# lh3/minimap2

Hardware: NVIDIA H100
Metric: aligned bases/sec (map-ont, 10 kb reads) (higher is better)
Workload: dtype int8 DP cells (int32 scores), u64 hashes, f32 chain penalties

## Files before the change

### include/mm_b200.h

```cpp
#ifndef MM_B200_H
#define MM_B200_H

#include <stdint.h>
#include <stddef.h>
#include "minimap.h"

#ifdef __cplusplus
extern "C" {
#endif

typedef struct mmb_ctx_s mmb_ctx_t;

int  mmb_device_count(void);
mmb_ctx_t *mmb_ctx_create(int device);
void mmb_ctx_destroy(mmb_ctx_t *ctx);
void *mmb_ctx_stream(mmb_ctx_t *ctx);
uint64_t mmb_launch_count(mmb_ctx_t *ctx, int reset);
void  mmb_profile_enable(mmb_ctx_t *ctx, int on);
double mmb_profile_ms(mmb_ctx_t *ctx, int which, int reset);
uint64_t mmb_profile_units(mmb_ctx_t *ctx, int which, int reset);

#define MMB_KSW_SCORE_ONLY   0x01
#define MMB_KSW_RIGHT        0x02
#define MMB_KSW_GENERIC_SC   0x04
// ... 23 lines not shown
} mmb_ksw_job_t;

typedef struct {
	int32_t max, zdropped;
	int32_t max_q, max_t;
	int32_t mqe, mqe_t;
	int32_t mte, mte_q;
	int32_t score;
	int32_t n_cigar, reach_end;
	uint32_t cigar_off;
	int32_t zd_max, zd_t0, zd_t1, zd_q0, zd_q1;
} mmb_ksw_res_t;

typedef struct {
	int8_t mat[25];
	int8_t q, e, q2, e2;
	int8_t noncan, junc_bonus, junc_pen;
	int16_t zd_skip;
} mmb_ksw_score_t;

int64_t mmb_ksw_batch_host(mmb_ctx_t *ctx, const mmb_ksw_score_t *sc, int n_jobs, const mmb_ksw_job_t *jobs,
						   const uint8_t *query, int64_t query_len, const uint8_t *target, int64_t target_len,
						   mmb_ksw_res_t *res, uint32_t *cigar_buf, int64_t cigar_cap);

int64_t mmb_sketch_batch_host(mmb_ctx_t *ctx, int n_seq, const char *seqs, const int64_t *off, int w, int k, int is_hpc,
							  uint32_t rid0, uint64_t *out_xy , int64_t out_cap, int64_t *n_out);

int mmb_ctx_set_junctions(mmb_ctx_t *ctx, int64_t n, const int64_t *st, const int64_t *en, const int8_t *strand);

int mmb_ctx_set_splice_scores(mmb_ctx_t *ctx, int strand, int64_t n, const int64_t *pos, const uint8_t *val);

typedef struct {
	int32_t max_dist_x, max_dist_y, bw, max_skip, max_iter, min_cnt, min_sc;
	float chn_pen_gap, chn_pen_skip;
	int32_t is_cdna, n_seg;
	int32_t use_rmq, max_dist_inner, rmq_size_cap;
} mmb_chain_par_t;

int mmb_chain_batch_host(mmb_ctx_t *ctx, const mmb_chain_par_t *par, int n_reads, const uint64_t *anchors_xy, const int64_t *a_off,
						 int32_t *n_u, int32_t *n_v, uint64_t *u_out, uint64_t *a_out_xy);
int mmb_chain_rmq_batch_host(mmb_ctx_t *ctx, const mmb_chain_par_t *par, int n_reads, const uint64_t *anchors_xy, const int64_t *a_off,
							 int32_t *n_u, int32_t *n_v, uint64_t *u_out, uint64_t *a_out_xy);

typedef struct {
	int64_t q0;
	int64_t t0;
// ... 57 lines not shown
```

### minimap2_b200/csrc/ksw_extd2.cu

```cuda
#include "mmb_internal.h"
#include "ksw_plan.h"
#include <algorithm>
#include <numeric>
#include <mutex>

#define KSW_NEG_INF (-0x40000000)

namespace {

struct KswArgs {
	const mmb_ksw_job_t *jobs;
	const int *order;
	int n;
	const uint8_t *query;
	const void *target;
	int t_packed;
	mmb_ksw_res_t *res;
	uint32_t *cigar;
	long long cigar_cap;
	unsigned long long *cigar_used;
	uint8_t *pws;
	size_t pws_stride;
	uint32_t *cigws;
	size_t cigws_stride;
// ... 696 lines not shown
		}
		uint64_t c = 0; for (int i : fastj) c += (uint64_t)h_jobs[i].qlen * h_jobs[i].tlen;
		fprintf(stderr, "[ksw] packed path: %zu jobs, cells %.3g; ll %zu\n", fastj.size(), (double)c, llj.size());
	}
	if (!tj[n_tiers].empty() || !tj[2 * n_tiers + 1].empty()) {
		fprintf(stderr, "[ERROR] ksw job longer than %d not supported by this build\n", tiers[n_tiers - 1].maxlen);
		abort();
	}
	if (!llj.empty()) {
		LLArgs L;
		int maxq = 1;
		for (int i : llj) maxq = std::max(maxq, h_jobs[i].qlen);
		L.jobs = d_jobs, L.query = d_query, L.target = d_target, L.t_packed = t_packed, L.res = d_res, L.n = (int)llj.size();
		for (int i = 0; i < 25; ++i) L.mat[i] = sc->mat[i];
		L.slen_max = (maxq + 7) / 8;
		L.ws_stride = ((size_t)L.slen_max * 8 * 2 * 4 + (size_t)L.slen_max * 8 + 255) & ~(size_t)255;
		int groups = std::min((int)llj.size(), ctx->n_sm * 16 * 4);
		int grid = (groups * 8 + 127) / 128;
		groups = grid * 16;
		int *d_order = (int*)ctx->d_g.reserve(((size_t)n_jobs * 3 + 256) * sizeof(int)) + (size_t)n_jobs * 2 + 128;
		L.counter = d_order, L.order = d_order + 1;
		K.ll.pws_bytes = L.ws_stride * (size_t)groups;
		K.ll.order = std::move(llj), K.ll.d_order = d_order;
		K.ll.go = [=](uint8_t *ws, uint32_t *) {
			LLArgs B = L;
			B.ws = (int16_t*)ws;
			ksw_ll_kernel<<<grid, 128, 0, ctx->stream>>>(B);
			MMB_CUDA_CHECK(cudaGetLastError());
			++ctx->n_launch;
		};
	}
	if (ctx->profiling) ctx->prof_bytes[MMB_PROF_KSW] += io_bytes + cells;
	int *d_queues = (int*)ctx->d_g.reserve(((size_t)n_jobs * 3 + 256) * sizeof(int));
	size_t g_off = (size_t)n_jobs + 64;
	std::vector<KswPlan> &plans = K.plans;
	K.cells = cells;
	mmb_ksw_fast_plan(ctx, sc, fastj, h_jobs, d_jobs, d_query, d_target, t_packed, d_res, d_cigar, cigar_cap, d_cigar_used, d_queues, plans);
	for (int pass = 0; pass < 2; ++pass) {
		if (pass == 1) {
			A.q = sc->q, A.e = sc->e, A.q2 = sc->q2, A.e2 = 0;
			A.skip = (-min_sc > 2 * (sc->q + sc->e)) || sc->q2 <= sc->q + sc->e;
			int lt2 = sc->e > 0? (sc->q2 - sc->q) / sc->e - 1 : 0;
			if (sc->q2 > sc->q + sc->e + lt2 * sc->e) ++lt2;
			A.long_thres = lt2, A.long_diff = lt2 * sc->e - (sc->q2 - sc->q);
		}
	for (int k = 0; k < n_tiers; ++k) {
		std::vector<int> &v = tj[pass * (n_tiers + 1) + k];
		if (v.empty()) continue;
		mmb_order_by_cells(v, h_jobs);
		int maxq = 0, maxt = 0; size_t maxp = 0; int maxsum = 0;
// ... 20 lines not shown
				MMB_CUDA_CHECK(cudaFuncSetAttribute(ksw_extd2_kernel<256, true>, cudaFuncAttributeMaxDynamicSharedMemorySize, (int)ctx->smem_optin - 1024));
			});
		}
		void (*kern)(KswArgs) = G == 32? (pass? ksw_extd2_kernel<32, true> : ksw_extd2_kernel<32, false>) : (pass? ksw_extd2_kernel<256, true> : ksw_extd2_kernel<256, false>);
		MMB_CUDA_CHECK(cudaOccupancyMaxActiveBlocksPerMultiprocessor(&cta_per_sm, kern, threads, smem));
		if (smem > ctx->smem_optin - 1024 || cta_per_sm < 1) {
			fprintf(stderr, "[ERROR] ksw tier %d needs %zu B shared memory per CTA\n", k, smem);
			abort();
		}
		int grid = ctx->n_sm * cta_per_sm;
		int need = ((int)v.size() + nw - 1) / nw;
		grid = std::max(1, std::min(grid, need));
		maxp = (maxp + 255) & ~(size_t)255;
		const size_t gws_stride = gstate? (state_bytes + 255) & ~(size_t)255 : 0;
		while ((size_t)grid * nw * (maxp + gws_stride) > ((size_t)2 << 30) && grid > 1) grid = (grid + 1) / 2;
		A.pws_stride = maxp, A.cigws_stride = (size_t)maxsum + 8;
		int *d_order = d_queues + g_off; g_off += v.size() + 1;
		A.counter = d_order, A.order = d_order + 1, A.n = (int)v.size();
		KswPlan pl;
		pl.order = std::move(v), pl.d_order = d_order;
		const size_t pws_area = A.pws_stride * (size_t)grid * nw;
		pl.pws_bytes = pws_area + gws_stride * (size_t)grid * nw, pl.cigws_bytes = A.cigws_stride * 4 * (size_t)grid * nw;
		const KswArgs A0 = A;
		pl.go = [=](uint8_t *pws, uint32_t *cigws) {
			KswArgs B = A0;
			B.pws = pws, B.cigws = cigws;
			B.gws = gstate? pws + pws_area : nullptr, B.gws_stride = gws_stride;
			kern<<<grid, threads, smem, ctx->stream>>>(B);
			MMB_CUDA_CHECK(cudaGetLastError());
			++ctx->n_launch;
		};
		plans.push_back(pl);
	}
	}
}

void mmb_ksw_enqueue(mmb_ctx_t *ctx, const KswLaunch &K)
{
	size_t pws_bytes = K.ll.pws_bytes, cigws_bytes = 0;
	for (const KswPlan &pl : K.plans) pws_bytes = std::max(pws_bytes, pl.pws_bytes), cigws_bytes = std::max(cigws_bytes, pl.cigws_bytes);
	uint8_t *pws = (uint8_t*)ctx->d_e.reserve(pws_bytes);
	uint32_t *cigws = (uint32_t*)ctx->d_f.reserve(cigws_bytes);
	auto upload = [&](const KswPlan &pl) {
		MMB_CUDA_CHECK(cudaMemcpyAsync(pl.d_order + 1, pl.order.data(), pl.order.size() * sizeof(int), cudaMemcpyHostToDevice, ctx->stream));
		MMB_CUDA_CHECK(cudaMemsetAsync(pl.d_order, 0, sizeof(int), ctx->stream));
	};
	if (K.ll.go) {
		upload(K.ll);
		ProfScope prof(ctx, MMB_PROF_OTHER, 0);
		K.ll.go(pws, nullptr);
	}
	for (const KswPlan &pl : K.plans) upload(pl);
	ProfScope prof(ctx, MMB_PROF_KSW, K.cells);
	for (const KswPlan &pl : K.plans) pl.go(pws, cigws);
}

void mmb_ksw_launch(mmb_ctx_t *ctx, const mmb_ksw_score_t *sc, int n_jobs, const mmb_ksw_job_t *h_jobs, const mmb_ksw_job_t *d_jobs,
					const uint8_t *d_query, const void *d_target, int t_packed,
					mmb_ksw_res_t *d_res, uint32_t *d_cigar, int64_t cigar_cap, unsigned long long *d_cigar_used)
{
	if (n_jobs <= 0) return;
	KswLaunch K;
	mmb_ksw_plan(ctx, sc, n_jobs, h_jobs, d_jobs, d_query, d_target, t_packed, d_res, d_cigar, cigar_cap, d_cigar_used, K);
	mmb_ksw_enqueue(ctx, K);
}
```

### minimap2_b200/csrc/ksw_fast.cu

```cuda
#include "mmb_internal.h"
#include "ksw_plan.h"
#include <algorithm>

#define KSW_NEG_INF (-0x40000000)

namespace {

struct FastArgs {
	const mmb_ksw_job_t *jobs;
	const int *order;
	int n;
	const uint8_t *query;
	const void *target;
	int t_packed;
	mmb_ksw_res_t *res;
	uint32_t *cigar;
	long long cigar_cap;
	unsigned long long *cigar_used;
	uint8_t *pws; size_t pws_stride;
	uint32_t *cigws; size_t cigws_stride;
	int *counter;
	int qmax;
	int8_t mch, mis, scn;
	int8_t q, e, q2, e2;
	int qe0;
	int8_t zd_q, zd_e;
	int8_t zd_scn;
	int zd_skip;
	int long_thres, long_diff;
	int8_t mat[25];
	uint32_t one, neg1;
};

__device__ __forceinline__ uint8_t fetch_t(const void *target, int packed, long long idx)
{
	if (packed) {
		const uint32_t *S = (const uint32_t*)target;
		return (uint8_t)(S[idx >> 3] >> ((idx & 7) << 2) & 0xf);
	}
	return ((const uint8_t*)target)[idx];
}

__device__ __forceinline__ void push_cig(uint32_t *cig, int &n, uint32_t op, int len)
{
	if (n == 0 || op != (cig[n - 1] & 0xf)) cig[n++] = (uint32_t)len << 4 | op;
	else cig[n - 1] += (uint32_t)len << 4;
}

template<int C>
__global__ void __launch_bounds__(128) ksw_fast_kernel(FastArgs A)
{
	extern __shared__ __align__(16) uint8_t smem[];
	const int lane = threadIdx.x & 31, wk = threadIdx.x >> 5, nwk = blockDim.x >> 5;
	const int worker = blockIdx.x * nwk + wk;
// ... 157 lines not shown
			if (jj >= 0) push_cig(cig, n, 1, jj + 1);
		}
		n = __shfl_sync(full, n, 0);
		unsigned long long coff = 0;
		if (n > 0) {
			if (lane == 0) coff = atomicAdd(A.cigar_used, (unsigned long long)n);
			coff = __shfl_sync(full, coff, 0);
			const bool rev_cigar = (jb.flag & MMB_KSW_REV_CIGAR) != 0;
			if ((long long)(coff + n) <= A.cigar_cap)
				for (int k = lane; k < n; k += 32) A.cigar[coff + k] = rev_cigar? cig[k] : cig[n - 1 - k];
		}
		if (lane == 0) {
			mmb_ksw_res_t o;
			o.zd_max = -1, o.zd_t0 = o.zd_t1 = o.zd_q0 = o.zd_q1 = -1;
			o.max = 0, o.zdropped = 0, o.max_q = o.max_t = o.mqe_t = o.mte_q = -1, o.mqe = o.mte = KSW_NEG_INF;
			o.score = score, o.n_cigar = n, o.reach_end = 0, o.cigar_off = (uint32_t)coff;
			A.res[jid] = o;
		}
		__syncwarp();
	}
}


#if defined(MMB_EMU) || defined(MMB_PK_NO_FMA)
#define PK_FADD(x, y) ((x) + (y))
#define PK_FSUB(x, y) ((x) - (y))
#else
#define PK_FADD(x, y) pk_mad((x), ONE, (y))
#define PK_FSUB(x, y) pk_mad((y), NEG1, (x))
__device__ __forceinline__ uint32_t pk_mad(uint32_t a, uint32_t b, uint32_t c)
{
	uint32_t d;
	asm("mad.lo.u32 %0, %1, %2, %3;" : "=r"(d) : "r"(a), "r"(b), "r"(c));
	return d;
}
#endif

template<int H, int LN>
#ifndef PK_MINB
#define PK_MINB (H <= 8? 4 : 3)
#endif
__global__ void __launch_bounds__(128, PK_MINB) ksw_pk_kernel(FastArgs A)
{
	extern __shared__ __align__(16) uint8_t smem[];
	constexpr int C = 2 * H;
	constexpr int CPH = H <= 1? 1 : H <= 2? 2 : H <= 4? 4 : H <= 8? 8 : 16;
// ... 6 lines not shown
	const int worker0 = (blockIdx.x * nwk + wk) * NJ;
	uint8_t *qs = smem + (size_t)(wk * NJ + grp) * A.qmax;
	constexpr int TSM = LN * C;
	constexpr int TW = 80, TILE = 32 * TW;
	uint8_t *ts = smem + (size_t)nwk * NJ * A.qmax + (size_t)(wk * NJ + grp) * TSM;
	uint8_t *tile = smem + (size_t)nwk * NJ * (A.qmax + TSM) + (size_t)wk * TILE;
	uint8_t *p = A.pws + A.pws_stride * (size_t)(worker0 + grp);
	const int q = A.q, e = A.e, q2 = A.q2, e2 = A.e2, qe = q + e, qe2 = q2 + e2;
	const unsigned full = 0xffffffffu;
	#define PK_ENC(v) ((uint32_t)((v) + 128) << 8)
	#define PK2(v) (PK_ENC(v) * 0x10001u)
	const uint32_t BB2 = 0x80008000u, CLEAN = 0xff00ff00u;
	const uint32_t TAGS = 0x03040506u, NBB2 = 0u - BB2;
	const uint32_t ONE = A.one, NEG1 = A.neg1;
	(void)ONE; (void)NEG1;
	const uint32_t KX = BB2 - ((uint32_t)e << 8) * 0x10001u - 0x00060006u, KY = BB2 - ((uint32_t)e << 8) * 0x10001u - 0x00050005u;
	const uint32_t KX2 = BB2 - ((uint32_t)e2 << 8) * 0x10001u - 0x00040004u, KY2 = BB2 - ((uint32_t)e2 << 8) * 0x10001u - 0x00030003u;
	const uint32_t NQX = PK2(-qe) | 0x00080008u, NQY = PK2(-qe) | 0x00100010u, NQX2 = PK2(-qe2) | 0x00200020u, NQY2 = PK2(-qe2) | 0x00400040u;
	const uint32_t SCN_T = PK2((int)A.scn) + 0x00070007u;
	const uint32_t KMM = (uint32_t)((int)A.mch - (int)A.mis) << 8;
	const uint32_t E_QE = PK_ENC(-q - e), E_E = PK_ENC(-e), E_E2 = PK_ENC(-e2), E_LD = PK_ENC(A.long_diff), E_QE2 = PK_ENC(-q2 - e2);
	const uint32_t XT0 = E_QE | 6u, YT0 = E_QE | 5u, X2T0 = E_QE2 | 4u, Y2T0 = E_QE2 | 3u;
	const int lt = A.long_thres;

	#pragma unroll 1
	for (;;) {
		int slot = 0;
		if (sub == 0) slot = atomicAdd(A.counter, 1);
		slot = __shfl_sync(full, slot, lead);
		const bool act = slot < A.n;
		if (!__any_sync(full, act)) break;
		int jid = -1, qlen = 0, tlen = 0, jflag = 0;
		mmb_ksw_job_t jb;
		if (act) { jid = A.order[slot]; jb = A.jobs[jid]; qlen = jb.qlen, tlen = jb.tlen, jflag = jb.flag; }
		for (int i = sub; i <= qlen; i += LN) {
			uint8_t c = 4;
			if (i < qlen) {
				c = A.query[jb.q_start + (long long)i * jb.q_step];
				if ((jflag & MMB_JOB_Q_COMP) && c < 4) c = 3 - c;
			}
			qs[i] = c < 4? (uint8_t)(1u << c) : (uint8_t)0x80;
		}
		const int t0 = sub * C;
		uint32_t TBM[H], MSC[H], U[H], Y[H], Y2[H];
		#pragma unroll
		for (int c = 0; c < H; ++c) {
			uint32_t tbm = 0, msc = 0, u = 0;
			#pragma unroll
			for (int h = 0; h < 2; ++h) {
// ... 92 lines not shown
						if constexpr (CPH == 1) *pa = (uint8_t)lo[0];
						else if constexpr (CPH == 2) *(uint16_t*)pa = (uint16_t)lo[0];
						else if constexpr (CPH == 4) *(uint32_t*)pa = lo[0];
						else if constexpr (CPH == 8) *(uint2*)pa = make_uint2(lo[0], lo[NW - 1]);
						else *(uint4*)pa = make_uint4(lo[0], lo[1], lo[2], lo[NW - 1]);
					}
					if (jA >= 1) {
						uint8_t *pb = pa + CPH;
						if constexpr (CPH == 1) *pb = (uint8_t)hi[0];
						else if constexpr (CPH == 2) *(uint16_t*)pb = (uint16_t)hi[0];
						else if constexpr (CPH == 4) *(uint32_t*)pb = hi[0];
						else if constexpr (CPH == 8) *(uint2*)pb = make_uint2(hi[0], hi[NW - 1]);
						else *(uint4*)pb = make_uint4(hi[0], hi[1], hi[2], hi[NW - 1]);
					}
				}
			}
		}
		int score = hrow;
		#pragma unroll
		for (int o = LN / 2; o > 0; o >>= 1) score += __shfl_xor_sync(full, score, o);
		score += (int)(hcol_acc >> 8) - 128 * qlen - A.qe0;
		score = __shfl_sync(full, score, lead);
		__syncwarp();
		#pragma unroll 1
		for (int g = 0; g < NJ; ++g) {
			const int src = g * LN;
			if (!__shfl_sync(full, (int)act, src)) continue;
			const int g_tlen = __shfl_sync(full, tlen, src), g_qlen = __shfl_sync(full, qlen, src), g_jid = __shfl_sync(full, jid, src);
			const int g_flag = __shfl_sync(full, jflag, src), g_score = __shfl_sync(full, score, src);
			const uint8_t *gp = A.pws + A.pws_stride * (size_t)(worker0 + g);
			uint32_t *cig = A.cigws + A.cigws_stride * (size_t)(worker0 + g);
			int n = 0, i = g_tlen - 1, jj = g_qlen - 1, state = 0;
			uint32_t run_op = 0, run_len = 0;
			int n_m = 0, gap_dp = 0, gap_zd = 0;
			#define PK_CLOSE() do { if (run_len) { if (run_op == 0) n_m += (int)run_len; else { const int l__c = (int)run_len; \
				gap_dp += min(q + e * l__c, q2 + e2 * l__c), gap_zd += A.zd_q + A.zd_e * l__c; } } } while (0)
			#define PK_EMIT(op_, len_) do { const uint32_t o__ = (op_), l__ = (len_); if (l__) { if (run_len && o__ == run_op) run_len += l__; \
				else { PK_CLOSE(); if (run_len && lane == 0) cig[n] = run_len << 4 | run_op; n += run_len? 1 : 0; run_op = o__, run_len = l__; } } } while (0)
			bool have = false;
			int tj = 0, tpb = 0;
			while (i >= 0 && jj >= 0) {
				const int di = (state == 0 || state == 1 || state == 3)? 1 : 0, dj = (state == 0 || state == 2 || state == 4)? 1 : 0;
				const int ci = i - lane * di, cj = jj - lane * dj;
				const bool inr = ci >= 0 && cj >= 0;
				int ph = 0, sr = 0;
				if (inr) { const int wi = ci % C, sb = ci / C; ph = sb * CP + (wi < H? wi : CPH + wi - H); sr = cj + 2 * sb + (wi < H? 0 : 1); }
// ... 18 lines not shown
				const bool cont = intile && (state == 0? (tmp & 7) == 0 : (tmp >> (state + 2) & 1) != 0);
				const unsigned stop = __ballot_sync(full, !cont);
				const int r = stop? __ffs(stop) - 1 : 32;
				PK_EMIT(state == 0? 0u : di? 2u : 1u, (uint32_t)r);
				i -= r * di, jj -= r * dj;
				if (r < 32) {
					const uint32_t tr = __shfl_sync(full, tmp, r);
					const bool in_r = __shfl_sync(full, (int)inr, r) != 0, in_t = __shfl_sync(full, (int)intile, r) != 0;
					if (!in_r) break;
					if (!in_t) continue;
					if (state == 0) {
						state = tr & 7;
						if (state == 1 || state == 3) { PK_EMIT(2u, 1u); --i; } else { PK_EMIT(1u, 1u); --jj; }
					} else state = 0;
				}
			}
			if (i >= 0) PK_EMIT(2u, (uint32_t)(i + 1));
			if (jj >= 0) PK_EMIT(1u, (uint32_t)(jj + 1));
			PK_CLOSE();
			if (run_len) { if (lane == 0) cig[n] = run_len << 4 | run_op; ++n; }
			#undef PK_EMIT
			#undef PK_CLOSE
			__syncwarp();
			int zd_max = -1, zd_t0 = -1, zd_t1 = -1, zd_q0 = -1, zd_q1 = -1;
			const bool zd_skip = A.zd_skip > 0 && A.mch * n_m - gap_dp - g_score + gap_zd <= A.zd_skip;
			if ((g_flag & MMB_JOB_ZDROP) && zd_skip) zd_max = 0;
			else if (g_flag & MMB_JOB_ZDROP) {
				const uint8_t *gq = smem + (size_t)(wk * NJ + g) * A.qmax;
				const uint8_t *gt = smem + (size_t)nwk * NJ * A.qmax + (size_t)(wk * NJ + g) * TSM;
				const int zq = A.zd_q, ze = A.zd_e, mch = A.mch, mis = A.mis, scn = A.zd_scn;
				int sco = 0, mx = INT32_MIN, mi = -1, mj = -1, ti0 = 0, qj0 = 0;
				zd_max = 0;
				for (int k = n - 1; k >= 0; --k) {
					const uint32_t op = cig[k] & 0xf; const int len = (int)(cig[k] >> 4);
					if (op == 0) {
						for (int base = 0; base < len; base += 32) {
							const bool valid = base + lane < len;
							const int ti = ti0 + base + lane, qj = qj0 + base + lane;
							int sc = 0;
							if (valid) {
								const uint32_t oh = gq[qj];
								const int tb = gt[ti];
								sc = (oh == 0x80 || tb == 4)? scn : (oh >> tb & 1)? mch : mis;
							}
							int S = sc;
							#pragma unroll
							for (int o = 1; o < 32; o <<= 1) { const int y = __shfl_up_sync(full, S, o); if (lane >= o) S += y; }
							S += sco;
// ... 14 lines not shown
							if (valid && !upd) { const int li = ti - cmi, lj = qj - cmj, diff = li > lj? li - lj : lj - li; z = M - S - diff * ze; }
							int zm = z;
							#pragma unroll
							for (int o = 16; o > 0; o >>= 1) zm = max(zm, __shfl_xor_sync(full, zm, o));
							if (zm > zd_max) {
								const int wl = __ffs(__ballot_sync(full, z == zm)) - 1;
								zd_max = zm, zd_t0 = __shfl_sync(full, cmi, wl), zd_t1 = __shfl_sync(full, ti, wl), zd_q0 = __shfl_sync(full, cmj, wl), zd_q1 = __shfl_sync(full, qj, wl);
							}
							const int L = __shfl_sync(full, lu, 31);
							if (L >= 0) mx = __shfl_sync(full, S, L), mi = ti0 + base + L, mj = qj0 + base + L;
							sco = __shfl_sync(full, S, min(32, len - base) - 1);
						}
						ti0 += len, qj0 += len;
					} else if (op == 1 || op == 2) {
						sco -= zq + ze * len;
						if (op == 1) qj0 += len; else ti0 += len;
						if (sco < mx) {
							const int li = ti0 - mi, lj = qj0 - mj, diff = li > lj? li - lj : lj - li, z = mx - sco - diff * ze;
							if (z > zd_max) zd_max = z, zd_t0 = mi, zd_t1 = ti0, zd_q0 = mj, zd_q1 = qj0;
						} else mx = sco, mi = ti0, mj = qj0;
					}
				}
			}
			unsigned long long coff = 0;
			if (n > 0) {
				if (lane == 0) coff = atomicAdd(A.cigar_used, (unsigned long long)n);
				coff = __shfl_sync(full, coff, 0);
				const bool rev_cigar = (g_flag & MMB_KSW_REV_CIGAR) != 0;
				if ((long long)(coff + n) <= A.cigar_cap)
					for (int k = lane; k < n; k += 32) A.cigar[coff + k] = rev_cigar? cig[k] : cig[n - 1 - k];
			}
			if (lane == 0) {
				mmb_ksw_res_t o;
				o.zd_max = -1, o.zd_t0 = o.zd_t1 = o.zd_q0 = o.zd_q1 = -1;
				o.max = 0, o.zdropped = 0, o.max_q = o.max_t = o.mqe_t = o.mte_q = -1, o.mqe = o.mte = KSW_NEG_INF;
				o.zd_max = zd_max, o.zd_t0 = zd_t0, o.zd_t1 = zd_t1, o.zd_q0 = zd_q0, o.zd_q1 = zd_q1;
				o.score = g_score, o.n_cigar = n, o.reach_end = 0, o.cigar_off = (uint32_t)coff;
				A.res[g_jid] = o;
			}
			__syncwarp();
		}
	}
	#undef PK_ENC
	#undef PK2
}

}

void mmb_order_by_cells(std::vector<int> &v, const mmb_ksw_job_t *h_jobs)
{
	const int NB = 40 * 16;
	auto key = [&](int i) {
		uint64_t c = (uint64_t)std::max(h_jobs[i].qlen, 1) * (uint64_t)std::max(h_jobs[i].tlen, 1);
		int lg = 63 - __builtin_clzll(c);
		int mant = lg >= 4? (int)(c >> (lg - 4)) & 15 : (int)(c << (4 - lg)) & 15;
		return NB - 1 - std::min(NB - 1, lg * 16 + mant);
	};
	std::vector<int> cnt(NB + 1, 0), out(v.size());
	for (int i : v) ++cnt[key(i) + 1];
	for (int b = 0; b < NB; ++b) cnt[b + 1] += cnt[b];
	for (int i : v) out[cnt[key(i)]++] = i;
	v.swap(out);
}

bool mmb_ksw_fast_eligible(const mmb_ksw_job_t &j)
{
	const int f = j.flag;
	if (f & (MMB_JOB_LL | MMB_JOB_SPLICE | MMB_JOB_T_COMP | MMB_KSW_SCORE_ONLY | MMB_KSW_RIGHT | MMB_KSW_APPROX_DROP | MMB_KSW_EXTZ_ONLY)) return false;
	if (!(f & MMB_KSW_APPROX_MAX)) return false;
	if (j.qlen <= 0 || j.tlen <= 0 || j.tlen > 512 || j.qlen > 2048) return false;
	const int w = j.w < 0? std::max(j.qlen, j.tlen) : j.w;
	return w >= std::max(j.qlen, j.tlen);
}

void mmb_ksw_fast_plan(mmb_ctx_t *ctx, const mmb_ksw_score_t *sc, const std::vector<int> &idx, const mmb_ksw_job_t *h_jobs, const mmb_ksw_job_t *d_jobs,
					   const uint8_t *d_query, const void *d_target, int t_packed, mmb_ksw_res_t *d_res, uint32_t *d_cigar, int64_t cigar_cap,
					   unsigned long long *d_cigar_used, int *d_order_all, std::vector<KswPlan> &plans)
{
	if (idx.empty()) return;
	FastArgs A;
	A.jobs = d_jobs, A.query = d_query, A.target = d_target, A.t_packed = t_packed, A.res = d_res;
	A.cigar = d_cigar, A.cigar_cap = cigar_cap, A.cigar_used = d_cigar_used;
	int8_t q = sc->q, e = sc->e, q2 = sc->q2, e2 = sc->e2;
	A.qe0 = q + e;
	if (q2 + e2 < q + e) std::swap(q, q2), std::swap(e, e2);
	A.q = q, A.e = e, A.q2 = q2, A.e2 = e2;
	A.zd_q = sc->q, A.zd_e = sc->e, A.zd_scn = sc->mat[24], A.zd_skip = sc->zd_skip;
	A.one = 1u, A.neg1 = 0xffffffffu;
	A.mch = sc->mat[0], A.mis = sc->mat[1], A.scn = sc->mat[24] == 0? (int8_t)(-e2) : sc->mat[24];
	for (int i = 0; i < 25; ++i) A.mat[i] = sc->mat[i];
	int lt = e != e2? (q2 - q) / (e - e2) - 1 : 0;
	if (q2 + e2 + lt * e2 > q + e + lt * e) ++lt;
	A.long_thres = lt, A.long_diff = lt * (e - e2) - (q2 - q) - e2;
	const int amax = std::max(std::abs((int)A.mch), std::max(std::abs((int)A.mis), std::abs((int)A.scn)));
	const bool pk_ok = 2 * std::max(q + e, q2 + e2) + amax + 8 <= 127 && A.mch > 0 && A.mis <= 0 && A.scn <= 0;
	static const int CW[] = { 2, 4, 6, 7, 8, 9, 10, 12, 14, 16,   4, 8, 12, 16, 20, 24,   14, 16 };
	static const int CPW[] = { 4, 4, 8, 8, 8, 16, 16, 16, 16, 16,   4, 8, 16, 16, 32, 32,   16, 16 };
	static const int LNW[] = { 32, 32, 32, 32, 32, 32, 32, 32, 32, 32,   16, 16, 16, 16, 16, 16,   32, 32 };
	const int NS = 10, NC = 18;
	std::vector<int> v[NC];
	for (int i : idx) {
		const bool pk = pk_ok && !(h_jobs[i].flag & MMB_KSW_GENERIC_SC);
		int k = pk? NS : 0;
		const int last = pk? NC - 1 : NS - 1;
		while (k < last && LNW[k] * CW[k] < h_jobs[i].tlen) ++k;
		v[k].push_back(i);
	}
	size_t order_off = 0;
	for (int k = 0; k < NC; ++k) {
		if (v[k].empty()) continue;
		mmb_order_by_cells(v[k], h_jobs);
// ... 12 lines not shown
		else if (k >= NS) switch (C) {
		case 14: kern = ksw_pk_kernel<7, 32>; break;  default: kern = ksw_pk_kernel<8, 32>; break;
		}
		else switch (C) {
		case 2: kern = ksw_fast_kernel<2>; break;   case 4: kern = ksw_fast_kernel<4>; break;
		case 6: kern = ksw_fast_kernel<6>; break;   case 7: kern = ksw_fast_kernel<7>; break;
		case 8: kern = ksw_fast_kernel<8>; break;   case 9: kern = ksw_fast_kernel<9>; break;
		case 10: kern = ksw_fast_kernel<10>; break; case 12: kern = ksw_fast_kernel<12>; break;
		case 14: kern = ksw_fast_kernel<14>; break; default: kern = ksw_fast_kernel<16>; break;
		}
		int cta_per_sm = 1;
		MMB_CUDA_CHECK(cudaOccupancyMaxActiveBlocksPerMultiprocessor(&cta_per_sm, kern, threads, smem));
		if (cta_per_sm < 1) { fprintf(stderr, "[ERROR] ksw_fast: no occupancy\n"); abort(); }
		int grid = ctx->n_sm * cta_per_sm;
		grid = std::max(1, std::min(grid, ((int)v[k].size() + nwk * NJ - 1) / (nwk * NJ)));
		A.pws_stride = ((size_t)(maxq + 2 * LNW[k] + 2) * W + 255) & ~(size_t)255;
		A.cigws_stride = (size_t)maxsum + 8;
		int *d_order = d_order_all + order_off; order_off += v[k].size() + 1;
		A.counter = d_order, A.order = d_order + 1, A.n = (int)v[k].size();
		KswPlan pl;
		pl.order = std::move(v[k]), pl.d_order = d_order;
		pl.pws_bytes = A.pws_stride * (size_t)grid * nwk * NJ + 256 , pl.cigws_bytes = A.cigws_stride * 4 * (size_t)grid * nwk * NJ;
		const FastArgs A0 = A;
		pl.go = [=](uint8_t *pws, uint32_t *cigws) {
			FastArgs B = A0;
			B.pws = pws, B.cigws = cigws;
			kern<<<grid, threads, smem, ctx->stream>>>(B);
			MMB_CUDA_CHECK(cudaGetLastError());
			++ctx->n_launch;
		};
		plans.push_back(pl);
	}
}
```

### minimap2_b200/csrc/ksw_plan.h

```cpp
#pragma once
#include <functional>
#include <vector>
#include <cstdint>
#include <cstddef>
struct KswPlan {
	size_t pws_bytes = 0, cigws_bytes = 0;
	std::vector<int> order;
	int *d_order = nullptr;
	std::function<void(uint8_t *pws, uint32_t *cigws)> go;
};
struct KswLaunch {
	KswPlan ll;
	std::vector<KswPlan> plans;
	uint64_t cells = 0;
};
void mmb_order_by_cells(std::vector<int> &v, const mmb_ksw_job_t *h_jobs);
void mmb_ksw_plan(mmb_ctx_t *ctx, const mmb_ksw_score_t *sc, int n_jobs, const mmb_ksw_job_t *h_jobs, const mmb_ksw_job_t *d_jobs,
				  const uint8_t *d_query, const void *d_target, int t_packed,
				  mmb_ksw_res_t *d_res, uint32_t *d_cigar, int64_t cigar_cap, unsigned long long *d_cigar_used, KswLaunch &K);
void mmb_ksw_enqueue(mmb_ctx_t *ctx, const KswLaunch &K);
```

### minimap2_b200/csrc/map.cu

```cuda
#include "pipeline.h"
#include "hostlogic.h"
#include "scan.cuh"
#include "ksw_plan.h"
#include "fastx.h"
#include <thread>
#include <unistd.h>
#include <malloc.h>
#include <climits>
#include <atomic>
#include <functional>
#include <cstring>
#include <algorithm>
#include <mutex>
#include <condition_variable>
#include <deque>
#include <memory>

extern "C" double realtime(void);
extern "C" double cputime(void);
int mmb_resident_reads(void);

namespace {

struct Task {
// ... 643 lines not shown
	mmb_stream_sync(ctx);
	ctx->last_h2d_bytes += in_bytes, ctx->last_d2h_bytes += out_bytes;
	HostSpan hs2_(ctx, HPH_TAIL_APPLY);
	const HlFinOut *h_fin = (const HlFinOut*)h_out;
	const uint32_t *h_fcig = (const uint32_t*)(h_out + sizeof(FinOut) * (size_t)n_hits);
	parallel_for((int64_t)nf, b.n_threads, [&](int64_t t, int) {
		hl_hp_flush();
		ReadState &r = rs[fr[t]];
		ReadAlign &ra = *r.ra;
		std::vector<const uint32_t*> cp(ra.fin_hits.size());
		for (size_t k = 0; k < cp.size(); ++k) cp[k] = h_fcig + coff[hoff[t] + k];
		int n_regs = r.n_regs;
		mm_reg1_t *regs = r.regs;
		bool ok;
		{ HpScope hp_(HP_EXTRA); ok = hl_align_apply_fin(ra, n_regs, regs, h_fin + hoff[t], cp.data()); }
		if (ok) hl_align_finish(b.opt, ra, &n_regs, regs);
		else {
			drop_regs(n_regs, regs);
			regs = replay_read(b, r, false, &n_regs);
			if (ra.incomplete) { fprintf(stderr, "[ERROR] minimap2_b200: host redo of a finished read is incomplete\n"); abort(); }
		}
		post_align(b, r, n_regs, regs);
	});
}

static int64_t ksw_wave(Batch &b, const std::vector<int> &active, const mmb_ksw_score_t &sc)
{
	mmb_ctx_t *ctx = b.ctx;
	BatchBufs &bb = b.bb;
	std::vector<ReadState> &rs = bb.rs_pool;
	std::vector<int64_t> joff(active.size() + 1, 0);
	for (size_t t = 0; t < active.size(); ++t) {
		ReadState &r = rs[active[t]];
		joff[t + 1] = joff[t] + (r.done? 0 : (int64_t)r.ra->want.size());
	}
	const int64_t n_jobs = joff[active.size()];
	if (n_jobs == 0) return 0;
	mmb_tl(ctx, MMB_TL_HOST_BEGIN, HPH_JOBS);
	if (b.wave >= 100000) { fprintf(stderr, "[ERROR] minimap2_b200: too many alignment waves\n"); abort(); }
	mmb_ksw_job_t *jobs = bb.h_jobs.as<mmb_ksw_job_t>((size_t)n_jobs);
	parallel_for((int64_t)active.size(), b.n_threads, [&](int64_t t, int) {
		ReadState &r = rs[active[t]];
		if (!r.done && !r.ra->want.empty()) memcpy(&jobs[joff[t]], r.ra->want.data(), sizeof(mmb_ksw_job_t) * r.ra->want.size());
	});
	static const int64_t CH = getenv("MM_B200_JOB_CHUNK")? std::max(1, atoi(getenv("MM_B200_JOB_CHUNK"))) : 1 << 20;
	mmb_ksw_res_t *res = bb.h_res.as<mmb_ksw_res_t>((size_t)n_jobs);
// ... 41 lines not shown
			const unsigned long long used = *h_used;
			if ((int64_t)used > cap) { cap = (int64_t)used + 16; gatew.drop(); continue; }
			if (cig_fill + (int64_t)used > cap_tot) {
				int64_t rest = 0;
				for (int64_t i = c0 + m; i < n_jobs; ++i) rest += cig_est(jobs[i]);
				const int64_t new_tot = cig_fill + (int64_t)used + rest + 64;
				std::unique_ptr<PinBuf> nb(new PinBuf);
				uint32_t *np_ = nb->as<uint32_t>((size_t)new_tot + 64);
				if (cig_fill) memcpy(np_, h_cig, (size_t)cig_fill * 4);
				bb.h_cig[b.wave]->release();
				bb.h_cig[b.wave] = std::move(nb);
				h_cig = np_, cap_tot = new_tot;
			}
			ctx->last_d2h_bytes += sizeof(mmb_ksw_res_t) * (uint64_t)m + 4ull * used;
			ctx->last_h2d_bytes += sizeof(mmb_ksw_job_t) * (uint64_t)m;
			if (ctx->profiling) ctx->prof_bytes[MMB_PROF_KSW] += 4ull * used;
			chunk_base.push_back(cig_fill);
			chunk_dev.push_back(d_cig + 2);
			++b.keep_used;
			if (used) MMB_CUDA_CHECK(cudaMemcpyAsync(h_cig + cig_fill, d_cig + 2, used * 4, cudaMemcpyDeviceToHost, ctx->stream));
			cig_fill += (int64_t)used;
			mmb_stream_sync(ctx);
			gatew.drop();
			break;
		}
	}
	HostSpan hs_(ctx, HPH_SCATTER);
	parallel_for((int64_t)active.size(), b.n_threads, [&](int64_t t, int) {
		ReadState &r = rs[active[t]];
		if (r.done) return;
		ReadAlign &ra = *r.ra;
		for (size_t i = 0; i < ra.want.size(); ++i) {
			const int64_t jid = joff[t] + (int64_t)i;
			KswDone d; d.r = res[jid], d.cig = h_cig + chunk_base[jid / CH] + res[jid].cigar_off, d.dcig = chunk_dev[jid / CH] + res[jid].cigar_off;
			ra.done_idx[ra.want_slot[i]] = (int)ra.done.size();
			ra.done.push_back(d);
		}
	});
	return n_jobs;
}

static void align_waves(Batch &b)
{
	std::vector<ReadState> &rs = b.bb.rs_pool;
	const mmb_ksw_score_t sc = ksw_score(b.opt);
	std::vector<int> active;
// ... 448 lines not shown
```

### minimap2_b200/csrc/mmb_ctx.cu

```cuda
#include "mmb_internal.h"
#include <cstring>
#include <ctime>

int mm_verbose_dummy_anchor = 0;

extern "C" int mmb_device_count(void)
{
	int n = 0;
	cudaError_t err = cudaGetDeviceCount(&n);
	if (err != cudaSuccess) {
		fprintf(stderr, "[ERROR] minimap2_b200: no usable CUDA device (%s); there is no CPU fallback\n", cudaGetErrorString(err));
		return -1;
	}
	return n;
}

bool g_mmb_tl_on = false;
double mmb_tl_now()
{
	timespec ts;
	clock_gettime(CLOCK_MONOTONIC, &ts);
	return (double)ts.tv_sec + 1e-9 * (double)ts.tv_nsec;
}
extern "C" void mmb_timeline_enable(int on) { g_mmb_tl_on = on != 0; }
// ... 11 lines not shown
		fprintf(stderr, "[ERROR] minimap2_b200: cannot create a context on device %d (%d visible)\n", device, n);
		return nullptr;
	}
	mmb_ctx_t *c = new mmb_ctx_t();
	c->device = device;
	MMB_CUDA_CHECK(cudaSetDevice(device));
	cudaDeviceProp prop;
	MMB_CUDA_CHECK(cudaGetDeviceProperties(&prop, device));
	c->n_sm = prop.multiProcessorCount;
	c->smem_optin = prop.sharedMemPerBlockOptin;
	MMB_CUDA_CHECK(cudaStreamCreateWithFlags(&c->stream, cudaStreamNonBlocking));
	MMB_CUDA_CHECK(cudaEventCreate(&c->ev0));
	MMB_CUDA_CHECK(cudaEventCreate(&c->ev1));
	MMB_CUDA_CHECK(cudaEventCreate(&c->ev_sync));
	return c;
}

extern "C" void mmb_ctx_destroy(mmb_ctx_t *c)
{
	if (!c) return;
	cudaSetDevice(c->device);
	cudaStreamSynchronize(c->stream);
	c->d_a.release(); c->d_b.release(); c->d_c.release(); c->d_d.release();
	c->d_e.release(); c->d_f.release(); c->d_g.release(); c->d_h.release(); c->sk_pk.release(); c->sk_nm.release(); c->sk_misc.release(); c->scan_sums.release(); c->d_junc.release(); c->d_spsc[0].release(); c->d_spsc[1].release();
	cudaEventDestroy(c->ev0); cudaEventDestroy(c->ev1); cudaEventDestroy(c->ev_sync);
	cudaStreamDestroy(c->stream);
	delete c;
}

extern "C" void *mmb_ctx_stream(mmb_ctx_t *c) { return (void*)c->stream; }

extern "C" int mmb_ctx_set_splice_scores(mmb_ctx_t *c, int strand, int64_t n, const int64_t *pos, const uint8_t *val)
{
	if (strand < 0 || strand > 1) return -1;
	MMB_CUDA_CHECK(cudaSetDevice(c->device));
	MMB_CUDA_CHECK(cudaStreamSynchronize(c->stream));
	c->spsc_pos[strand] = nullptr, c->spsc_val[strand] = nullptr, c->n_spsc[strand] = 0;
	if (n <= 0) return 0;
	for (int64_t i = 1; i < n; ++i) if (pos[i] <= pos[i - 1]) return -1;
	uint8_t *d = (uint8_t*)c->d_spsc[strand].reserve((size_t)n * 9 + 64);
	MMB_CUDA_CHECK(cudaMemcpy(d, pos, (size_t)n * 8, cudaMemcpyHostToDevice));
	MMB_CUDA_CHECK(cudaMemcpy(d + (size_t)n * 8, val, (size_t)n, cudaMemcpyHostToDevice));
	c->spsc_pos[strand] = (const int64_t*)d, c->spsc_val[strand] = d + (size_t)n * 8, c->n_spsc[strand] = n;
	return 0;
}

extern "C" int mmb_ctx_set_junctions(mmb_ctx_t *c, int64_t n, const int64_t *st, const int64_t *en, const int8_t *strand)
{
// ... 50 lines not shown
{
	if (n_jobs <= 0) return 0;
	MMB_CUDA_CHECK(cudaSetDevice(ctx->device));
	uint8_t *d_q = ctx->d_a.as<uint8_t>(query_len + 16), *d_t = ctx->d_b.as<uint8_t>(target_len + 16);
	mmb_ksw_job_t *d_jobs = ctx->d_c.as<mmb_ksw_job_t>(n_jobs);
	mmb_ksw_res_t *d_res = ctx->d_d.as<mmb_ksw_res_t>(n_jobs);
	uint32_t *d_cig = (uint32_t*)ctx->d_h.reserve((size_t)(cigar_cap + 2) * 4 + 16);
	unsigned long long *d_used = (unsigned long long*)(d_cig);
	MMB_CUDA_CHECK(cudaMemcpyAsync(d_q, query, query_len, cudaMemcpyHostToDevice, ctx->stream));
	MMB_CUDA_CHECK(cudaMemcpyAsync(d_t, target, target_len, cudaMemcpyHostToDevice, ctx->stream));
	MMB_CUDA_CHECK(cudaMemcpyAsync(d_jobs, jobs, sizeof(mmb_ksw_job_t) * n_jobs, cudaMemcpyHostToDevice, ctx->stream));
	MMB_CUDA_CHECK(cudaMemsetAsync(d_used, 0, 8, ctx->stream));
	mmb_ksw_launch(ctx, sc, n_jobs, jobs, d_jobs, d_q, d_t, 0, d_res, d_cig + 2, cigar_cap, d_used);
	unsigned long long used = 0;
	MMB_CUDA_CHECK(cudaMemcpyAsync(res, d_res, sizeof(mmb_ksw_res_t) * n_jobs, cudaMemcpyDeviceToHost, ctx->stream));
	MMB_CUDA_CHECK(cudaMemcpyAsync(&used, d_used, 8, cudaMemcpyDeviceToHost, ctx->stream));
	MMB_CUDA_CHECK(cudaStreamSynchronize(ctx->stream));
	if ((int64_t)used > cigar_cap) return -(int64_t)used;
	MMB_CUDA_CHECK(cudaMemcpyAsync(cigar_buf, d_cig + 2, used * 4, cudaMemcpyDeviceToHost, ctx->stream));
	MMB_CUDA_CHECK(cudaStreamSynchronize(ctx->stream));
	return (int64_t)used;
}

mmb_ctx_t *mmb_default_ctx(void);
extern "C" void *mmb_default_ctx_c(void) { return (void*)mmb_default_ctx(); }
extern "C" void mmb_free(void *p) { free(p); }

extern "C" uint64_t mmb_profile_scopes(mmb_ctx_t *c, int which, int reset)
{
	if (which < 0 || which >= MMB_PROF_N) return 0;
	mmb_profile_ms(c, which, 0);
	uint64_t v = c->prof_launches[which];
	if (reset) c->prof_launches[which] = 0;
	return v;
}

extern "C" uint64_t mmb_profile_bytes(mmb_ctx_t *c, int which, int reset)
{
	if (which < 0 || which >= MMB_PROF_N) return 0;
	uint64_t v = c->prof_bytes[which];
	if (reset) c->prof_bytes[which] = 0;
	return v;
}
static int g_resident_reads = 0;
extern "C" void mmb_set_resident_reads(int on) { g_resident_reads = on; }
int mmb_resident_reads(void) { return g_resident_reads; }
// ... 52 lines not shown
```

### minimap2_b200/csrc/mmb_internal.h

```cpp
#pragma once
#include <cuda_runtime.h>
#include <cstdint>
#include <cstdio>
#include <cstdlib>
#include <vector>
#include <utility>
#include <chrono>
#include <thread>
#include "mm_b200.h"

extern "C" int mm_verbose;

#define MMB_CUDA_CHECK(expr) do { \
	cudaError_t err__ = (expr); \
	if (err__ != cudaSuccess) { \
		fprintf(stderr, "[ERROR] CUDA failure '%s' at %s:%d: %s\n", #expr, __FILE__, __LINE__, cudaGetErrorString(err__)); \
		abort(); \
	} } while (0)

enum { MMB_PROF_SKETCH = 0, MMB_PROF_SEED = 1, MMB_PROF_SORT = 2, MMB_PROF_CHAIN = 3, MMB_PROF_KSW = 4, MMB_PROF_OTHER = 5, MMB_PROF_N = 6 };

struct DevBuf {
	void *p = nullptr;
	size_t cap = 0;
// ... 6 lines not shown
		}
		return p;
	}
	template<class T> T *as(size_t n) { return (T*)reserve(n * sizeof(T)); }
	void release() { if (p) cudaFree(p); p = nullptr; cap = 0; }
};

struct PinBuf {
	void *p = nullptr;
	size_t cap = 0;
	void *reserve(size_t bytes) {
		if (bytes > cap) {
			if (p) MMB_CUDA_CHECK(cudaFreeHost(p));
			size_t ncap = bytes + (bytes >> 2) + 256;
			MMB_CUDA_CHECK(cudaMallocHost(&p, ncap));
			cap = ncap;
		}
		return p;
	}
	template<class T> T *as(size_t n) { return (T*)reserve(n * sizeof(T)); }
	void release() { if (p) cudaFreeHost(p); p = nullptr; cap = 0; }
};

struct mmb_ctx_s {
	int device = 0;
	int group_id = 0;
	int n_sm = 0;
	size_t smem_optin = 0;
	cudaStream_t stream = nullptr;
	uint64_t n_launch = 0;
	int profiling = 0;
	double prof_ms[MMB_PROF_N] = {0};
	uint64_t prof_units[MMB_PROF_N] = {0};
	cudaEvent_t ev0 = nullptr, ev1 = nullptr;
	std::vector<cudaEvent_t> ev_pool;
	std::vector<std::pair<cudaEvent_t, cudaEvent_t>> ev_pending[MMB_PROF_N];
	uint64_t prof_launches[MMB_PROF_N] = {0};
	uint64_t prof_bytes[MMB_PROF_N] = {0};
	uint64_t last_d2h_bytes = 0, last_h2d_bytes = 0;
	DevBuf d_a, d_b, d_c, d_d, d_e, d_f, d_g, d_h;
	DevBuf sk_pk, sk_nm, sk_misc, scan_sums;
	const int64_t *junc_st = nullptr, *junc_en = nullptr; const int8_t *junc_strand = nullptr; int64_t n_junc = 0;
	DevBuf d_junc;
	const int64_t *spsc_pos[2] = {nullptr, nullptr}; const uint8_t *spsc_val[2] = {nullptr, nullptr}; int64_t n_spsc[2] = {0, 0};
	DevBuf d_spsc[2];
	std::vector<double> tl;
	cudaEvent_t ev_sync = nullptr;
	bool sleepy_sync = false;
};

enum {
	MMB_TL_GATE_REQ = 0,
	MMB_TL_GATE_GRANT = 1,
	MMB_TL_GATE_REL = 2,
	MMB_TL_ENQUEUED = 3,
	MMB_TL_SYNC = 4,
	MMB_TL_HOST_BEGIN = 5,
	MMB_TL_HOST_END = 6,
};
extern bool g_mmb_tl_on;
double mmb_tl_now();
inline void mmb_tl(mmb_ctx_t *c, int ev, int arg = 0)
{
	if (g_mmb_tl_on) c->tl.push_back(mmb_tl_now()), c->tl.push_back(ev), c->tl.push_back(arg);
}
inline void mmb_stream_sync(mmb_ctx_t *c)
{
	if (c->sleepy_sync) {
		MMB_CUDA_CHECK(cudaEventRecord(c->ev_sync, c->stream));
		cudaError_t st;
		while ((st = cudaEventQuery(c->ev_sync)) == cudaErrorNotReady) std::this_thread::sleep_for(std::chrono::microseconds(20));
// ... 28 lines not shown
```

Baseline: 1.193 billion.

## Run extd2 KSW plans concurrently on side streams with separate workspaces

Marks each extd2 KSW tier plan as a side plan and gives it its own workspace slice, then launches these plans on up to three non-blocking side streams. The fast-path plans keep running on the main stream, and the main stream waits on events from the side streams afterwards. The goal is to let kernels from different length tiers overlap and fill the GPU instead of running one after another, at the cost of larger workspace allocations. The change also adds optional clock64 phase instrumentation to the fast kernel and an env-gated job dump, which add a per-lap null-pointer check.

After: 1.264 billion, median of 6. +6.0%, better.

```diff
diff --git a/include/mm_b200.h b/include/mm_b200.h
--- a/include/mm_b200.h
+++ b/include/mm_b200.h
@@ -69,6 +69,7 @@
 int64_t mmb_ksw_batch_host(mmb_ctx_t *ctx, const mmb_ksw_score_t *sc, int n_jobs, const mmb_ksw_job_t *jobs,
 						   const uint8_t *query, int64_t query_len, const uint8_t *target, int64_t target_len,
 						   mmb_ksw_res_t *res, uint32_t *cigar_buf, int64_t cigar_cap);
+void mmb_ksw_phase_clocks(mmb_ctx_t *ctx, int on, unsigned long long *out);
 
 int64_t mmb_sketch_batch_host(mmb_ctx_t *ctx, int n_seq, const char *seqs, const int64_t *off, int w, int k, int is_hpc,
 							  uint32_t rid0, uint64_t *out_xy , int64_t out_cap, int64_t *n_out);
diff --git a/minimap2_b200/csrc/ksw_extd2.cu b/minimap2_b200/csrc/ksw_extd2.cu
--- a/minimap2_b200/csrc/ksw_extd2.cu
+++ b/minimap2_b200/csrc/ksw_extd2.cu
@@ -742,10 +742,10 @@
 		L.counter = d_order, L.order = d_order + 1;
 		K.ll.pws_bytes = L.ws_stride * (size_t)groups;
 		K.ll.order = std::move(llj), K.ll.d_order = d_order;
-		K.ll.go = [=](uint8_t *ws, uint32_t *) {
+		K.ll.go = [=](uint8_t *ws, uint32_t *, cudaStream_t st) {
 			LLArgs B = L;
 			B.ws = (int16_t*)ws;
-			ksw_ll_kernel<<<grid, 128, 0, ctx->stream>>>(B);
+			ksw_ll_kernel<<<grid, 128, 0, st>>>(B);
 			MMB_CUDA_CHECK(cudaGetLastError());
 			++ctx->n_launch;
 		};
@@ -812,11 +812,12 @@
 		const size_t pws_area = A.pws_stride * (size_t)grid * nw;
 		pl.pws_bytes = pws_area + gws_stride * (size_t)grid * nw, pl.cigws_bytes = A.cigws_stride * 4 * (size_t)grid * nw;
 		const KswArgs A0 = A;
-		pl.go = [=](uint8_t *pws, uint32_t *cigws) {
+		pl.side = true;
+		pl.go = [=](uint8_t *pws, uint32_t *cigws, cudaStream_t st) {
 			KswArgs B = A0;
 			B.pws = pws, B.cigws = cigws;
 			B.gws = gstate? pws + pws_area : nullptr, B.gws_stride = gws_stride;
-			kern<<<grid, threads, smem, ctx->stream>>>(B);
+			kern<<<grid, threads, smem, st>>>(B);
 			MMB_CUDA_CHECK(cudaGetLastError());
 			++ctx->n_launch;
 		};
@@ -827,10 +828,14 @@
 
 void mmb_ksw_enqueue(mmb_ctx_t *ctx, const KswLaunch &K)
 {
-	size_t pws_bytes = K.ll.pws_bytes, cigws_bytes = 0;
-	for (const KswPlan &pl : K.plans) pws_bytes = std::max(pws_bytes, pl.pws_bytes), cigws_bytes = std::max(cigws_bytes, pl.cigws_bytes);
-	uint8_t *pws = (uint8_t*)ctx->d_e.reserve(pws_bytes);
-	uint32_t *cigws = (uint32_t*)ctx->d_f.reserve(cigws_bytes);
+	size_t pws_bytes = K.ll.pws_bytes, cigws_bytes = 0, side_pws = 0, side_cig = 0;
+	for (const KswPlan &pl : K.plans) {
+		if (pl.side) side_pws += (pl.pws_bytes + 255) & ~(size_t)255, side_cig += (pl.cigws_bytes + 255) & ~(size_t)255;
+		else pws_bytes = std::max(pws_bytes, pl.pws_bytes), cigws_bytes = std::max(cigws_bytes, pl.cigws_bytes);
+	}
+	pws_bytes = (pws_bytes + 255) & ~(size_t)255, cigws_bytes = (cigws_bytes + 255) & ~(size_t)255;
+	uint8_t *pws = (uint8_t*)ctx->d_e.reserve(pws_bytes + side_pws);
+	uint8_t *cigws = (uint8_t*)ctx->d_f.reserve(cigws_bytes + side_cig);
 	auto upload = [&](const KswPlan &pl) {
 		MMB_CUDA_CHECK(cudaMemcpyAsync(pl.d_order + 1, pl.order.data(), pl.order.size() * sizeof(int), cudaMemcpyHostToDevice, ctx->stream));
 		MMB_CUDA_CHECK(cudaMemsetAsync(pl.d_order, 0, sizeof(int), ctx->stream));
@@ -838,11 +843,42 @@
 	if (K.ll.go) {
 		upload(K.ll);
 		ProfScope prof(ctx, MMB_PROF_OTHER, 0);
-		K.ll.go(pws, nullptr);
+		K.ll.go(pws, nullptr, ctx->stream);
 	}
 	for (const KswPlan &pl : K.plans) upload(pl);
 	ProfScope prof(ctx, MMB_PROF_KSW, K.cells);
-	for (const KswPlan &pl : K.plans) pl.go(pws, cigws);
+	int n_side = 0;
+	for (const KswPlan &pl : K.plans) n_side += pl.side;
+#ifndef MMB_EMU
+	if (n_side && !ctx->ksw_side[0]) for (int k = 0; k < MMB_KSW_SIDE; ++k) {
+		MMB_CUDA_CHECK(cudaStreamCreateWithFlags(&ctx->ksw_side[k], cudaStreamNonBlocking));
+		MMB_CUDA_CHECK(cudaEventCreateWithFlags(&ctx->ksw_side_ev[k], cudaEventDisableTiming));
+	}
+	if (n_side) {
+		MMB_CUDA_CHECK(cudaEventRecord(ctx->ksw_side_ev[0], ctx->stream));
+		for (int k = 0; k < std::min(n_side, MMB_KSW_SIDE); ++k) MMB_CUDA_CHECK(cudaStreamWaitEvent(ctx->ksw_side[k], ctx->ksw_side_ev[0], 0));
+	}
+#endif
+	size_t po = pws_bytes, co = cigws_bytes;
+	int k_side = 0;
+	for (const KswPlan &pl : K.plans) {
+		if (!pl.side) continue;
+#ifdef MMB_EMU
+		cudaStream_t st = ctx->stream;
+#else
+		cudaStream_t st = ctx->ksw_side[k_side % MMB_KSW_SIDE];
+#endif
+		pl.go(pws + po, (uint32_t*)(cigws + co), st);
+		po += (pl.pws_bytes + 255) & ~(size_t)255, co += (pl.cigws_bytes + 255) & ~(size_t)255;
+		++k_side;
+	}
+	for (const KswPlan &pl : K.plans) if (!pl.side) pl.go(pws, (uint32_t*)cigws, ctx->stream);
+#ifndef MMB_EMU
+	for (int k = 0; k < std::min(n_side, MMB_KSW_SIDE); ++k) {
+		MMB_CUDA_CHECK(cudaEventRecord(ctx->ksw_side_ev[k], ctx->ksw_side[k]));
+		MMB_CUDA_CHECK(cudaStreamWaitEvent(ctx->stream, ctx->ksw_side_ev[k], 0));
+	}
+#endif
 }
 
 void mmb_ksw_launch(mmb_ctx_t *ctx, const mmb_ksw_score_t *sc, int n_jobs, const mmb_ksw_job_t *h_jobs, const mmb_ksw_job_t *d_jobs,
diff --git a/minimap2_b200/csrc/ksw_fast.cu b/minimap2_b200/csrc/ksw_fast.cu
--- a/minimap2_b200/csrc/ksw_fast.cu
+++ b/minimap2_b200/csrc/ksw_fast.cu
@@ -30,6 +30,7 @@
 	int long_thres, long_diff;
 	int8_t mat[25];
 	uint32_t one, neg1;
+	unsigned long long *clk;
 };
 
 __device__ __forceinline__ uint8_t fetch_t(const void *target, int packed, long long idx)
@@ -233,6 +234,9 @@
 }
 
 
+#ifdef MMB_EMU
+static inline long long clock64() { return 0; }
+#endif
 #if defined(MMB_EMU) || defined(MMB_PK_NO_FMA)
 #define PK_FADD(x, y) ((x) + (y))
 #define PK_FSUB(x, y) ((x) - (y))
@@ -285,9 +289,12 @@
 	const uint32_t E_QE = PK_ENC(-q - e), E_E = PK_ENC(-e), E_E2 = PK_ENC(-e2), E_LD = PK_ENC(A.long_diff), E_QE2 = PK_ENC(-q2 - e2);
 	const uint32_t XT0 = E_QE | 6u, YT0 = E_QE | 5u, X2T0 = E_QE2 | 4u, Y2T0 = E_QE2 | 3u;
 	const int lt = A.long_thres;
+	long long tlap = 0;
+	#define PK_LAP(k) do { if (A.clk && lane == 0) { const long long t__ = clock64(); atomicAdd(A.clk + (k), (unsigned long long)(t__ - tlap)); tlap = t__; } } while (0)
 
 	#pragma unroll 1
 	for (;;) {
+		if (A.clk) tlap = clock64();
 		int slot = 0;
 		if (sub == 0) slot = atomicAdd(A.counter, 1);
 		slot = __shfl_sync(full, slot, lead);
@@ -426,6 +433,7 @@
 		score += (int)(hcol_acc >> 8) - 128 * qlen - A.qe0;
 		score = __shfl_sync(full, score, lead);
 		__syncwarp();
+		PK_LAP(0);
 		#pragma unroll 1
 		for (int g = 0; g < NJ; ++g) {
 			const int src = g * LN;
@@ -490,8 +498,10 @@
 			#undef PK_EMIT
 			#undef PK_CLOSE
 			__syncwarp();
+			PK_LAP(1);
 			int zd_max = -1, zd_t0 = -1, zd_t1 = -1, zd_q0 = -1, zd_q1 = -1;
 			const bool zd_skip = A.zd_skip > 0 && A.mch * n_m - gap_dp - g_score + gap_zd <= A.zd_skip;
+			if (A.clk && lane == 0 && (g_flag & MMB_JOB_ZDROP)) atomicAdd(A.clk + (zd_skip? 5 : 4), 1ull);
 			if ((g_flag & MMB_JOB_ZDROP) && zd_skip) zd_max = 0;
 			else if (g_flag & MMB_JOB_ZDROP) {
 				const uint8_t *gq = smem + (size_t)(wk * NJ + g) * A.qmax;
@@ -552,6 +562,7 @@
 					}
 				}
 			}
+			PK_LAP(2);
 			unsigned long long coff = 0;
 			if (n > 0) {
 				if (lane == 0) coff = atomicAdd(A.cigar_used, (unsigned long long)n);
@@ -569,10 +580,12 @@
 				A.res[g_jid] = o;
 			}
 			__syncwarp();
+			PK_LAP(3);
 		}
 	}
 	#undef PK_ENC
 	#undef PK2
+	#undef PK_LAP
 }
 
 }
@@ -617,6 +630,7 @@
 	A.q = q, A.e = e, A.q2 = q2, A.e2 = e2;
 	A.zd_q = sc->q, A.zd_e = sc->e, A.zd_scn = sc->mat[24], A.zd_skip = sc->zd_skip;
 	A.one = 1u, A.neg1 = 0xffffffffu;
+	A.clk = ctx->ksw_clk;
 	A.mch = sc->mat[0], A.mis = sc->mat[1], A.scn = sc->mat[24] == 0? (int8_t)(-e2) : sc->mat[24];
 	for (int i = 0; i < 25; ++i) A.mat[i] = sc->mat[i];
 	int lt = e != e2? (q2 - q) / (e - e2) - 1 : 0;
@@ -675,10 +689,10 @@
 		pl.order = std::move(v[k]), pl.d_order = d_order;
 		pl.pws_bytes = A.pws_stride * (size_t)grid * nwk * NJ + 256 , pl.cigws_bytes = A.cigws_stride * 4 * (size_t)grid * nwk * NJ;
 		const FastArgs A0 = A;
-		pl.go = [=](uint8_t *pws, uint32_t *cigws) {
+		pl.go = [=](uint8_t *pws, uint32_t *cigws, cudaStream_t st) {
 			FastArgs B = A0;
 			B.pws = pws, B.cigws = cigws;
-			kern<<<grid, threads, smem, ctx->stream>>>(B);
+			kern<<<grid, threads, smem, st>>>(B);
 			MMB_CUDA_CHECK(cudaGetLastError());
 			++ctx->n_launch;
 		};
diff --git a/minimap2_b200/csrc/ksw_plan.h b/minimap2_b200/csrc/ksw_plan.h
--- a/minimap2_b200/csrc/ksw_plan.h
+++ b/minimap2_b200/csrc/ksw_plan.h
@@ -3,11 +3,13 @@
 #include <vector>
 #include <cstdint>
 #include <cstddef>
+#include <cuda_runtime.h>
 struct KswPlan {
 	size_t pws_bytes = 0, cigws_bytes = 0;
 	std::vector<int> order;
 	int *d_order = nullptr;
-	std::function<void(uint8_t *pws, uint32_t *cigws)> go;
+	bool side = false;
+	std::function<void(uint8_t *pws, uint32_t *cigws, cudaStream_t st)> go;
 };
 struct KswLaunch {
 	KswPlan ll;
diff --git a/minimap2_b200/csrc/map.cu b/minimap2_b200/csrc/map.cu
--- a/minimap2_b200/csrc/map.cu
+++ b/minimap2_b200/csrc/map.cu
@@ -689,6 +689,37 @@
 		}
 		post_align(b, r, n_regs, regs);
 	});
+}
+
+static void ksw_dump(const char *path, const Batch &b, const mmb_ksw_job_t *jobs, int64_t m)
+{
+	static std::mutex mu;
+	static std::vector<uint32_t> S;
+	std::lock_guard<std::mutex> lk(mu);
+	if (S.empty()) {
+		const mm_idx_seq_t &last = b.mi->seq[b.mi->n_seq - 1];
+		S.resize((last.offset + last.len + 7) / 8 + 1);
+		MMB_CUDA_CHECK(cudaMemcpy(S.data(), b.mi->B->d_S, (S.size() - 1) * 4, cudaMemcpyDeviceToHost));
+	}
+	std::vector<uint8_t> seq((size_t)b.total_bases);
+	MMB_CUDA_CHECK(cudaMemcpy(seq.data(), b.d_seq, seq.size(), cudaMemcpyDeviceToHost));
+	std::vector<mmb_ksw_job_t> out(jobs, jobs + m);
+	std::vector<uint8_t> qb, tb;
+	for (mmb_ksw_job_t &j : out) {
+		const int64_t q0 = std::min(j.q_start, j.q_start + (int64_t)(j.qlen - 1) * j.q_step), t0 = std::min(j.t_start, j.t_start + (int64_t)(j.tlen - 1) * j.t_step);
+		const int64_t qo = (int64_t)qb.size(), to = (int64_t)tb.size();
+		for (int k = 0; k < j.qlen; ++k) qb.push_back(seq[q0 + k]);
+		for (int k = 0; k < j.tlen; ++k) tb.push_back((uint8_t)(S[(t0 + k) >> 3] >> (((t0 + k) & 7) << 2) & 0xf));
+		j.q_start = qo + (j.q_start - q0), j.t_start = to + (j.t_start - t0);
+	}
+	FILE *fp = fopen(path, "ab");
+	if (!fp) { fprintf(stderr, "[ERROR] cannot open %s\n", path); abort(); }
+	const int64_t hdr[3] = { m, (int64_t)qb.size(), (int64_t)tb.size() };
+	fwrite(hdr, sizeof(hdr), 1, fp);
+	fwrite(out.data(), sizeof(mmb_ksw_job_t), out.size(), fp);
+	fwrite(qb.data(), 1, qb.size(), fp);
+	fwrite(tb.data(), 1, tb.size(), fp);
+	fclose(fp);
 }
 
 static int64_t ksw_wave(Batch &b, const std::vector<int> &active, const mmb_ksw_score_t &sc)
@@ -776,6 +807,8 @@
 			cig_fill += (int64_t)used;
 			mmb_stream_sync(ctx);
 			gatew.drop();
+			static const char *dump_path = getenv("MM_B200_KSW_DUMP");
+			if (dump_path) ksw_dump(dump_path, b, &jobs[c0], m);
 			break;
 		}
 	}
diff --git a/minimap2_b200/csrc/mmb_ctx.cu b/minimap2_b200/csrc/mmb_ctx.cu
--- a/minimap2_b200/csrc/mmb_ctx.cu
+++ b/minimap2_b200/csrc/mmb_ctx.cu
@@ -57,8 +57,9 @@
 	cudaSetDevice(c->device);
 	cudaStreamSynchronize(c->stream);
 	c->d_a.release(); c->d_b.release(); c->d_c.release(); c->d_d.release();
-	c->d_e.release(); c->d_f.release(); c->d_g.release(); c->d_h.release(); c->sk_pk.release(); c->sk_nm.release(); c->sk_misc.release(); c->scan_sums.release(); c->d_junc.release(); c->d_spsc[0].release(); c->d_spsc[1].release();
+	c->d_e.release(); c->d_f.release(); c->d_g.release(); c->d_h.release(); c->d_clk.release(); c->sk_pk.release(); c->sk_nm.release(); c->sk_misc.release(); c->scan_sums.release(); c->d_junc.release(); c->d_spsc[0].release(); c->d_spsc[1].release();
 	cudaEventDestroy(c->ev0); cudaEventDestroy(c->ev1); cudaEventDestroy(c->ev_sync);
+	for (int k = 0; k < MMB_KSW_SIDE; ++k) if (c->ksw_side[k]) cudaStreamDestroy(c->ksw_side[k]), cudaEventDestroy(c->ksw_side_ev[k]);
 	cudaStreamDestroy(c->stream);
 	delete c;
 }
@@ -155,6 +156,19 @@
 	return (int64_t)used;
 }
 
+extern "C" void mmb_ksw_phase_clocks(mmb_ctx_t *c, int on, unsigned long long *out)
+{
+	MMB_CUDA_CHECK(cudaSetDevice(c->device));
+	MMB_CUDA_CHECK(cudaStreamSynchronize(c->stream));
+	if (on) {
+		c->ksw_clk = c->d_clk.as<unsigned long long>(8);
+		MMB_CUDA_CHECK(cudaMemset(c->ksw_clk, 0, 8 * sizeof(unsigned long long)));
+		return;
+	}
+	if (out && c->ksw_clk) MMB_CUDA_CHECK(cudaMemcpy(out, c->ksw_clk, 6 * sizeof(unsigned long long), cudaMemcpyDeviceToHost));
+	c->ksw_clk = nullptr;
+}
+
 mmb_ctx_t *mmb_default_ctx(void);
 extern "C" void *mmb_default_ctx_c(void) { return (void*)mmb_default_ctx(); }
 extern "C" void mmb_free(void *p) { free(p); }
diff --git a/minimap2_b200/csrc/mmb_internal.h b/minimap2_b200/csrc/mmb_internal.h
--- a/minimap2_b200/csrc/mmb_internal.h
+++ b/minimap2_b200/csrc/mmb_internal.h
@@ -52,6 +52,7 @@
 	void release() { if (p) cudaFreeHost(p); p = nullptr; cap = 0; }
 };
 
+#define MMB_KSW_SIDE 3
 struct mmb_ctx_s {
 	int device = 0;
 	int group_id = 0;
@@ -77,6 +78,10 @@
 	std::vector<double> tl;
 	cudaEvent_t ev_sync = nullptr;
 	bool sleepy_sync = false;
+	cudaStream_t ksw_side[MMB_KSW_SIDE] = {};
+	cudaEvent_t ksw_side_ev[MMB_KSW_SIDE] = {};
+	unsigned long long *ksw_clk = nullptr;
+	DevBuf d_clk;
 };
 
 enum {
```
